# monniert/differentiable-blocksworld

Measured on AMD Instinct MI355X. Metric: rendered views/sec (fwd+bwd) per node, DTU 400x300 K=10 blocks, higher is better.
Workload: dtype f32; 1 GPU; DTU-scan24-like synthetic: 49 views/GPU/step, 400x300, 10 superquadric blocks + ground + sky dome, faces_per_pixel=10, 256^2 textures, coarse phase (sigma=1e-4, opacity noise, decimated textures), MSE+parsimony+TV+overlap, Adam; LPIPS excluded; views_per_gpu=49, n_blocks=10, faces_per_pixel=10, txt_size=256, parallelism=one GPU: all views on it, no collective, nranks=1

## Files before the change

differentiable-blocksworld_amd/csrc/model_ops.hip:

```cpp
#include "dbw_common.h"
#include "model_math.h"
#include "rng_math.h"
#include "texture_body.h"
#include "step_kernels.h"
#include "../../include/dbw_hip.h"

using namespace dbw;

namespace {

__device__ __forceinline__ int dense_index(const int *keep, int k) {
    if (!keep) return k;
    int c = 0;
    for (int i = 0; i < k; ++i) c += keep[i] != 0;
    return c;
}

__global__ __launch_bounds__(64) void sq_blocks_fwd_kernel(const float *sq_eps, const float *S, const float *R6, const float *T,
                                                           const float *trig, const int *keep, int dense, int Kb, int nv, float ratio,
                                                           float scale_min, float S_world, const float *Rw, const float *Tw,
                                                           float *verts) {
    const int k = blockIdx.x;
    if (keep && !keep[k]) {
        if (!dense)
// ... 31 lines not shown
        float loc[3], de1[3], de2[3];
        parametric_sq_point(trig[o], trig[plane + o], trig[2 * plane + o], trig[3 * plane + o], p.e1, p.e2, ratio, loc, de1, de2);
        float gv[3];
        pose_bwd(p, loc, S_world, Rw, gverts + ((long long)ko * nv + v) * 3, acc, gv);
        acc[0] += gv[0] * de1[0] + gv[1] * de1[1] + gv[2] * de1[2];
        acc[1] += gv[0] * de2[0] + gv[1] * de2[1] + gv[2] * de2[2];
    }
#pragma unroll
    for (int i = 0; i < 17; ++i) acc[i] = wave_sum(acc[i]);
    if (threadIdx.x == 0) finish_pose_grads(p, S, k, acc, g_sq_eps, g_S, g_R6, g_T);
}

__global__ __launch_bounds__(64) void posed_mesh_fwd_kernel(const float *base, int nv, const float *R6, const float *T,
                                                            float S_world, const float *Rw, const float *Tw, float *verts) {
    Pose p;
    load_pose(nullptr, nullptr, R6, T, 0, 0.f, p);
    for (int v = blockIdx.x * 64 + threadIdx.x; v < nv; v += gridDim.x * 64)
        pose_fwd(p, base + (long long)v * 3, S_world, Rw, Tw, verts + (long long)v * 3);
}

__global__ __launch_bounds__(64) void posed_mesh_bwd_kernel(const float *base, int nv, const float *R6, const float *T,
                                                            float S_world, const float *Rw, const float *gverts, float *g_R6,
                                                            float *g_T) {
    Pose p;
    load_pose(nullptr, nullptr, R6, T, 0, 0.f, p);
    float acc[17];
#pragma unroll
    for (int i = 0; i < 17; ++i) acc[i] = 0.f;
    for (int v = threadIdx.x; v < nv; v += 64) {
        float gv[3];
        pose_bwd(p, base + (long long)v * 3, S_world, Rw, gverts + (long long)v * 3, acc, gv);
    }
#pragma unroll
    for (int i = 0; i < 17; ++i) acc[i] = wave_sum(acc[i]);
    if (threadIdx.x == 0) finish_pose_grads(p, nullptr, 0, acc, nullptr, nullptr, g_R6, g_T);
}

constexpr int MAX_KB = 64;
constexpr int NG = 18;

struct BlockP {
    float e1, e2, sr[3], R[9], T[3], alpha;
};

struct OverlapShared { BlockP b[MAX_KB]; float g[MAX_KB * NG]; float red[4]; };
__device__ __forceinline__ void overlap_block(const float *u, unsigned long long seed, unsigned long long rng_step, int npts, const float *sq_eps,
                                              const float *S, const float *R6, const float *T, const float *alpha, int Kb, float ratio,
                                              float scale_min, float inv_temp, float thresh, float scale_over_P, float *loss, float *ws,
                                              OverlapShared &sh) {
    BlockP *s_b = sh.b;
    float *s_g = sh.g, *s_red = sh.red;
    for (int j = threadIdx.x; j < Kb; j += blockDim.x) {
        Pose p;
        load_pose(sq_eps, S, R6, T, j, scale_min, p);
        BlockP &b = s_b[j];
        b.e1 = p.e1; b.e2 = p.e2; b.alpha = alpha[j];
        for (int i = 0; i < 3; ++i) { b.sr[i] = p.S[i] * ratio; b.T[i] = p.T[i]; b.R[i] = p.rot.b1[i]; b.R[3 + i] = p.rot.b2[i]; b.R[6 + i] = p.rot.b3[i]; }
    }
// ... 354 lines not shown
```

differentiable-blocksworld_amd/csrc/project_clip.hip:

```cpp
#include "dbw_common.h"
#include "camera_math.h"
#include "shade_common.h"
#include "raster_bin.h"
#include "step_kernels.h"
#include "texture_body.h"
#include "../../include/dbw_hip.h"

using namespace dbw;

namespace {

constexpr int NT = 256;

__device__ __forceinline__ void store_tri(float *dst, f3 a, f3 b, f3 c) {
    dst[0] = a.x; dst[1] = a.y; dst[2] = a.z;
    dst[3] = b.x; dst[4] = b.y; dst[5] = b.z;
    dst[6] = c.x; dst[7] = c.y; dst[8] = c.z;
}

__global__ __launch_bounds__(NT) void project_clip_fwd_kernel(
    const float *__restrict__ verts, const int *__restrict__ faces, const float *__restrict__ R,
    const float *__restrict__ T, const float *__restrict__ Kmat, int V, int F, float eps, int zc_on, float zc,
    int persp, float *__restrict__ fvc, int *__restrict__ first_idx, int *__restrict__ num_faces,
    int *__restrict__ c2o, int *__restrict__ neighbor, int *__restrict__ code, float *__restrict__ cw) {
// ... 19 lines not shown
        const int prefix = __popcll(m1 & lower) + __popcll(m2 & lower);
        if (lane == 0) s_wcnt[wv] = __popcll(m1) + __popcll(m2);
        __syncthreads();
        int woff = 0, tot = 0;
#pragma unroll
        for (int w = 0; w < NT / DBW_WAVE; ++w) { const int c = s_wcnt[w]; if (w < wv) woff += c; tot += c; }
        const int slot = running + woff + prefix;
        if (emit >= 1) {
            const long long o = base_out + slot;
            store_tri(fvc + o * 9, cf.t0[0], cf.t0[1], cf.t0[2]);
            c2o[o] = f; neighbor[o] = emit == 2 ? (int)(o + 1) : -1; code[o] = cf.code0; cw[o * 2] = cf.w2; cw[o * 2 + 1] = cf.w3;
            if (emit == 2) {
                store_tri(fvc + (o + 1) * 9, cf.t1[0], cf.t1[1], cf.t1[2]);
                c2o[o + 1] = f; neighbor[o + 1] = (int)o; code[o + 1] = cf.code1; cw[(o + 1) * 2] = cf.w2; cw[(o + 1) * 2 + 1] = cf.w3;
            }
        }
        running += tot;
        __syncthreads();
    }
    if (tid == 0) { first_idx[b] = (int)base_out; num_faces[b] = running; }
}

constexpr int BWD_SLOTS = 8;
template <bool LDS_TABLE>
__device__ __forceinline__ void project_clip_bwd_body(
    const float *__restrict__ verts, const int *__restrict__ faces, const float *__restrict__ R,
    const float *__restrict__ T, const float *__restrict__ Kmat, int B, int V, int F, float eps, float zc, int persp,
    const int *__restrict__ num_faces, const int *__restrict__ c2o, const int *__restrict__ code,
    const float *__restrict__ cw, const float *__restrict__ gfvc, float *gverts, float *s_acc, int blk) {
    const int lane = threadIdx.x & 63;
    if (LDS_TABLE) {
        for (int i = threadIdx.x; i < V * 3; i += NT) s_acc[i] = 0.f;
        __syncthreads();
    }
    constexpr int WAVES = NT / DBW_WAVE, ITERS = LDS_TABLE ? BWD_SLOTS / WAVES : 1;
    for (int it = 0; it < ITERS; ++it) {
    const int j = LDS_TABLE ? blk * BWD_SLOTS + it * WAVES + (threadIdx.x >> 6) : blk * WAVES + (threadIdx.x >> 6);
    if (j >= 2 * F) break;
    for (int b0 = 0; b0 < B; b0 += DBW_WAVE) {
        const int b = b0 + lane;
        bool act = b < B && j < num_faces[b];
        const long long o = (long long)(act ? b : 0) * 2 * F + j;
        float g[9];
        if (act) {
            bool any = false;
#pragma unroll
            for (int i = 0; i < 9; ++i) { g[i] = gfvc[o * 9 + i]; any |= (g[i] != 0.f); }
            act = any;
        }
        int f = -1, vi[3] = {0, 0, 0};
        float gw[9] = {0.f, 0.f, 0.f, 0.f, 0.f, 0.f, 0.f, 0.f, 0.f};
        if (act) {
            Cam cam;
            load_cam(R, T, Kmat, b, cam);
            f = c2o[o];
            const int cd = code[o];
            vi[0] = faces[f * 3]; vi[1] = faces[f * 3 + 1]; vi[2] = faces[f * 3 + 2];
            f3 gv[3] = {{0.f, 0.f, 0.f}, {0.f, 0.f, 0.f}, {0.f, 0.f, 0.f}};
            const f3 ga{g[0], g[1], g[2]}, gb{g[3], g[4], g[5]}, gc{g[6], g[7], g[8]};
            if (cd < 0) {
                gv[0] = ga; gv[1] = gb; gv[2] = gc;
            } else {
                const int i1 = cd & 3, kind = cd >> 2;
                const f3 q0 = project(verts + (long long)vi[0] * 3, cam, eps).ndc, q1 = project(verts + (long long)vi[1] * 3, cam, eps).ndc,
                         q2 = project(verts + (long long)vi[2] * 3, cam, eps).ndc;
                const f3 P1 = i1 == 0 ? q0 : (i1 == 1 ? q1 : q2), P2 = i1 == 0 ? q1 : (i1 == 1 ? q2 : q0),
                         P3 = i1 == 0 ? q2 : (i1 == 1 ? q0 : q1);
                const float w2 = cw[o * 2], w3 = cw[o * 2 + 1];
                f3 g1{0.f, 0.f, 0.f}, g2{0.f, 0.f, 0.f}, g3{0.f, 0.f, 0.f};
                if (kind == 0) {
                    clip_point_bwd(P1, P2, zc, persp, w2, ga, g1, g2);
                    clip_point_bwd(P1, P3, zc, persp, w3, gb, g1, g3);
                    g1.x += gc.x; g1.y += gc.y; g1.z += gc.z;
                } else if (kind == 1) {
                    clip_point_bwd(P1, P2, zc, persp, w2, ga, g1, g2);
                    g2.x += gb.x; g2.y += gb.y; g2.z += gb.z;
                    clip_point_bwd(P1, P3, zc, persp, w3, gc, g1, g3);
                } else {
                    clip_point_bwd(P1, P3, zc, persp, w3, ga, g1, g3);
                    g2.x += gb.x; g2.y += gb.y; g2.z += gb.z;
                    g3.x += gc.x; g3.y += gc.y; g3.z += gc.z;
                }
                gv[0] = i1 == 0 ? g1 : (i1 == 1 ? g3 : g2);
                gv[1] = i1 == 0 ? g2 : (i1 == 1 ? g1 : g3);
                gv[2] = i1 == 0 ? g3 : (i1 == 1 ? g2 : g1);
            }
#pragma unroll
            for (int i = 0; i < 3; ++i)
                if (gv[i].x != 0.f || gv[i].y != 0.f || gv[i].z != 0.f) {
                    const f3 w = vertex_bwd(verts, vi[i], cam, eps, gv[i]);
                    gw[i * 3] = w.x; gw[i * 3 + 1] = w.y; gw[i * 3 + 2] = w.z;
                }
        }
        const unsigned long long am = __ballot(act);
        if (am == 0ull) continue;
        const int leader = __ffsll((long long)am) - 1;
        const int f0 = __shfl(f, leader, 64);
        if (__popcll(am) >= 4 && __ballot(act && f == f0) == am) {
            float s[9];
#pragma unroll
            for (int c = 0; c < 9; ++c) s[c] = wave_sum_dpp(gw[c]);
            if (lane == leader) {
#pragma unroll
                for (int c = 0; c < 9; ++c)
                    if (s[c] != 0.f) {
                        if (LDS_TABLE) atomicAdd(&s_acc[vi[c / 3] * 3 + (c % 3)], s[c]);
                        else unsafeAtomicAdd(gverts + (long long)vi[c / 3] * 3 + (c % 3), s[c]);
                    }
            }
        } else if (act) {
#pragma unroll
            for (int c = 0; c < 9; ++c)
                if (gw[c] != 0.f) {
                    if (LDS_TABLE) atomicAdd(&s_acc[vi[c / 3] * 3 + (c % 3)], gw[c]);
                    else unsafeAtomicAdd(gverts + (long long)vi[c / 3] * 3 + (c % 3), gw[c]);
                }
        }
    }
    }
    if (LDS_TABLE) {
        __syncthreads();
        for (int i = threadIdx.x; i < V * 3; i += NT) {
            const float v = s_acc[i];
            if (v != 0.f) unsafeAtomicAdd(gverts + i, v);
        }
    }
}

template <bool LDS_TABLE>
__global__ __launch_bounds__(NT) void project_clip_bwd_kernel(
    const float *__restrict__ verts, const int *__restrict__ faces, const float *__restrict__ R,
    const float *__restrict__ T, const float *__restrict__ Kmat, int B, int V, int F, float eps, float zc, int persp,
    const int *__restrict__ num_faces, const int *__restrict__ c2o, const int *__restrict__ code,
    const float *__restrict__ cw, const float *__restrict__ gfvc, float *__restrict__ gverts) {
    extern __shared__ float s_acc[];
    project_clip_bwd_body<LDS_TABLE>(verts, faces, R, T, Kmat, B, V, F, eps, zc, persp, num_faces, c2o, code, cw, gfvc, gverts, s_acc, blockIdx.x);
}

template <bool LDS_TABLE>
__global__ __launch_bounds__(NT) void clip_bwd_tex_kernel(const ClipBwdArgs C, const dbw_texture_set t, int nclip) {
    extern __shared__ float s_acc[];
    if ((int)blockIdx.x < nclip)
        project_clip_bwd_body<LDS_TABLE>(C.verts, C.faces, C.R, C.T, C.Kmat, C.B, C.V, C.F, C.eps, C.zc, C.persp, C.num_faces, C.c2o, C.code, C.cw, C.gfvc,
                                         C.gverts, s_acc, blockIdx.x);
    else
        texture_prep_bwd_body(t.texture, t.n, t.h, t.w, t.decim, t.grad_maps, t.grad_sig, t.grad_texture, (long long)blockIdx.x - nclip,
                              (long long)gridDim.x - nclip);
}

template <bool CACHED>
__global__ __launch_bounds__(NT) void scene_setup_kernel(const SceneSetupArgs A) {
    __shared__ int s_wcnt[NT / DBW_WAVE];
    extern __shared__ float s_ndc[];
    if (A.sync_flag && blockIdx.x == 0 && blockIdx.y == 0 && blockIdx.z == 0 && threadIdx.x == 0)
        __hip_atomic_store(A.sync_flag, A.sync_val, __ATOMIC_RELEASE, __HIP_MEMORY_SCOPE_AGENT);
    const SceneGeom &G = A.sc[A.scene0 + blockIdx.z];
    const int chunk = blockIdx.x, b = blockIdx.y, tid = threadIdx.x, lane = tid & 63, wv = tid >> 6;
    const int F = G.F, nchunks = (F + NT - 1) / NT;
    if (chunk >= nchunks) return;
    if (G.hdr && chunk == 0 && b == 0)
        for (int i = tid; i < G.nhdr; i += NT) G.hdr[i] = 0;
    Cam cam;
    load_cam(A.R, A.T, A.Kmat, b, cam);
    const long long base_out = (long long)b * 2 * F;
    const int f = chunk * NT + tid;
    int vi[3] = {0, 0, 0};
    if (f < F) { vi[0] = G.faces[f * 3]; vi[1] = G.faces[f * 3 + 1]; vi[2] = G.faces[f * 3 + 2]; }
    if (CACHED) {
        for (int v = tid; v < G.V; v += NT) {
            const f3 q = project(G.verts + (long long)v * 3, cam, G.cam_eps).ndc;
// ... 79 lines not shown
            srec[0] = sr;
        }
    }
}

}

int dbw::launch_clip_bwd_tex(const ClipBwdArgs &C, const dbw_texture_set &t, hipStream_t s) {
    DBW_REQUIRE(C.verts && C.faces && C.R && C.T && C.Kmat && C.num_faces && C.c2o && C.code && C.cw && C.gfvc && C.gverts, "null pointer");
    DBW_REQUIRE(C.B > 0 && C.V > 0 && C.F > 0, "bad size");
    DBW_REQUIRE(t.texture && t.grad_maps && t.grad_texture && t.n > 0 && t.h > 0 && t.w > 0 && t.decim >= 1, "bad texture set");
    const long long work = (long long)t.n * t.h * t.w * 3;
    long long ntex = (work + NT - 1) / NT;
    if (ntex > 4096) ntex = 4096;
    const bool table = (size_t)C.V * 3 * sizeof(float) <= 48 * 1024;
    const int nclip = table ? (2 * C.F + BWD_SLOTS - 1) / BWD_SLOTS : (2 * C.F + NT / DBW_WAVE - 1) / (NT / DBW_WAVE);
    if (table)
        hipLaunchKernelGGL(clip_bwd_tex_kernel<true>, dim3((unsigned)(nclip + ntex)), dim3(NT), (size_t)C.V * 3 * sizeof(float), s, C, t, nclip);
    else
        hipLaunchKernelGGL(clip_bwd_tex_kernel<false>, dim3((unsigned)(nclip + ntex)), dim3(NT), 0, s, C, t, nclip);
    return dbw_check_launch("clip_bwd_tex_kernel");
}

int dbw::launch_scene_setup(const SceneSetupArgs &A, hipStream_t s) {
    DBW_REQUIRE(A.R && A.T && A.Kmat && A.B > 0, "bad argument");
    int chunks = 0;
    DBW_REQUIRE(A.scene0 >= 0 && A.nscenes >= 1 && A.scene0 + A.nscenes <= 2, "bad scene range");
    for (int i = A.scene0; i < A.scene0 + A.nscenes; ++i) {
        const SceneGeom &G = A.sc[i];
        DBW_REQUIRE(G.verts && G.faces && G.fvc && G.first_idx && G.num_faces && G.c2o && G.neighbor && G.code && G.cw && G.bbox && G.recs, "null pointer");
        DBW_REQUIRE(G.V > 0 && G.F > 0 && (long long)A.B * 2 * G.F < 0x7fffffffLL && (!G.zc_on || G.zc > 0.f), "bad size / z_clip");
        DBW_REQUIRE(!G.srec || (G.face_uvs && G.face_map && G.map_desc), "null pointer");
        chunks = max(chunks, (G.F + NT - 1) / NT);
    }
    int vmax = 0;
    for (int i = A.scene0; i < A.scene0 + A.nscenes; ++i) vmax = max(vmax, A.sc[i].V);
    if ((size_t)vmax * 12 <= 40 * 1024)
        hipLaunchKernelGGL(scene_setup_kernel<true>, dim3((unsigned)chunks, (unsigned)A.B, (unsigned)A.nscenes), dim3(NT), (size_t)vmax * 12, s, A);
    else
        hipLaunchKernelGGL(scene_setup_kernel<false>, dim3((unsigned)chunks, (unsigned)A.B, (unsigned)A.nscenes), dim3(NT), 0, s, A);
    return dbw_check_launch("scene_setup_kernel");
}

extern "C" int dbw_project_clip_fwd(const float *verts_world, const int32_t *faces, const float *R, const float *T,
                                    const float *Kmat, int B, int V, int F, float eps, int z_clip_enabled,
                                    float z_clip, int perspective_correct, float *face_verts_c, int32_t *first_idx,
// ... 34 lines not shown
```

differentiable-blocksworld_amd/csrc/step_kernels.h:

```cpp
#pragma once
#include <hip/hip_runtime.h>
#include <stdint.h>

#include "../../include/dbw_hip.h"

namespace dbw {
struct RasterWorkspace;

constexpr int STEP_MAX_SETS = 4;
struct StepTextureSets { dbw_texture_set s[STEP_MAX_SETS]; };

struct PrologueArgs {
    StepTextureSets tex; int nsets;
    const float *alpha_logit, *noise;
    float noise_scale, thresh;
    int nb;
    float *alpha, *alpha_full;
    int *keep;
    unsigned long long seed, rng_step;
    const float *sq_eps, *S, *R6, *T, *trig;
    int nv;
    float ratio, scale_min, S_world;
    const float *Rw, *Tw;
    float *blk_verts;
// ... 41 lines not shown
    float pars_eps, pars_scale;
    float *loss_parsimony, *loss_overlap;
    float *g_sq_eps, *g_S, *g_R6, *g_T, *g_alpha_full;
    float *ws;
    unsigned *ticket;
};
int launch_regularisers(const RegulariserArgs &A, hipStream_t s);

struct BlocksTailArgs {
    const float *sq_eps, *S, *R6, *T, *sq_local; const int *keep; int nb, nv; float scale_min, S_world; const float *Rw;
    const float *g_verts;
    float *g_sq_eps, *g_S, *g_R6, *g_T;
    const float *alpha, *g_alpha_parts, *g_alpha_full; int alpha_parts; float *g_logit;
    const float *void_raised; float *void_flag;
};
int launch_blocks_tail(const BlocksTailArgs &A, hipStream_t s);

struct ClipBwdArgs {
    const float *verts; const int *faces; const float *R, *T, *Kmat; int B, V, F; float eps, zc; int persp;
    const int *num_faces, *c2o, *code; const float *cw, *gfvc; float *gverts;
};
int launch_clip_bwd_tex(const ClipBwdArgs &C, const dbw_texture_set &tex, hipStream_t s);

struct AdamTailArgs {
    float *param, *grad, *exp_avg, *exp_avg_sq; const int64_t *group_end; const float *lr; int ngroups;
    float beta1, beta2, eps; int step;
    void *zero_buf; int64_t zero_bytes, hole_begin, hole_end;
    dbw_texture_set tex[2]; int ntex;
    const float *void_raised; float *void_flag;
};
bool adam_tail_fits(const AdamTailArgs &A);
int launch_adam_tail(const AdamTailArgs &A, hipStream_t s);

struct EnvFoldHost {
    const RasterWorkspace *ws; const int *first_idx, *num_faces; const float *maps; float bg[3];
    int *p2f; float *uvj;
};
int render_fwd_fused_mse_fold(const float *face_verts_c, const int32_t *first_idx, const int32_t *num_faces, const int32_t *neighbor,
                              const int32_t *c2o, const int32_t *clip_code, const float *clip_w, int Fc_stride, const float *face_uvs,
                              const int32_t *face_map, const int32_t *map_desc, const float *maps, const float *faces_alpha, int alpha_len, int N,
                              int64_t F_total, int H, int W, int K, int F, float sigma, float blur_radius, int perspective_correct,
                              const float *background3, int32_t *pix_to_face, float *bary, float *dists, void *workspace, size_t workspace_bytes,
                              const float *target, float mse_scale, float *loss_partial, float *grad_fg, float *grad_env, const EnvFoldHost &fold,
                              float *rec_out, const float *grad_rec, hipStream_t stream);

int render_bwd_fused_signal(const int32_t *pix_to_face, const float *bary, const float *dists, const int32_t *c2o, const int32_t *clip_code,
// ... 9 lines not shown
```

differentiable-blocksworld_amd/csrc/train_step.hip:

```cpp
#include "dbw_common.h"
#include "raster_bin.h"
#include "step_kernels.h"
#include "../../include/dbw_hip.h"

#include <math.h>
#include <mutex>
#include <new>
#include <stdlib.h>
#include <string.h>

using namespace dbw;

namespace {

__global__ __launch_bounds__(256) void tile_target_kernel(const float *__restrict__ img, int B, int C, int H, int W, float *__restrict__ out) {
    const int tx = (W + 7) >> 3, ty = (H + 7) >> 3;
    const long long total = (long long)B * ty * tx * C * 64;
    for (long long i = (long long)blockIdx.x * blockDim.x + threadIdx.x; i < total; i += (long long)gridDim.x * blockDim.x) {
        const int lane = (int)(i & 63);
        long long r = i >> 6;
        const int c = (int)(r % C); r /= C;
        const int tix = (int)(r % tx); r /= tx;
        const int tiy = (int)(r % ty);
        const int n = (int)(r / ty);
// ... 237 lines not shown

struct dbw_step_plan {
    dbw_step_desc d;
    Layout L;
    char *ws;
    RasterWorkspace rw_e, rw_f;
    hipEvent_t ev_prologue, ev_scatter, ev_fg_fwd, ev_reg, ev_layout, ev_kernel_done, ev_blocks_ready, ev_env_done, ev_losses;
    hipStream_t stream_r, stream_env;
    unsigned long long runs;
    int bin_turn, bin_ready, uniform_ready;
    bool arena_clean;
    float *host_losses;
    bool losses_pending;
    bool phase1_done;
    bool cur_flags;
    bool profile, profiled;
    hipEvent_t ev_t[8];
    unsigned *sync_words;
    unsigned *host_timeouts, *host_timeouts_dev;
    unsigned sync_val[SYNC_FLAGS];
    int voided_runs;
    int force_timeout;
    bool last_tail;
};

extern "C" size_t dbw_train_step_workspace_bytes(const dbw_step_desc *desc) {
    if (check_desc(desc)) return 0;
    Layout L;
    make_layout(*desc, L);
    return L.total;
}

extern "C" dbw_step_plan *dbw_train_step_create(const dbw_step_desc *desc, void *workspace, size_t workspace_bytes) {
    if (check_desc(desc)) return nullptr;
    if (!workspace || ((uintptr_t)workspace & 255)) { dbw_set_error("dbw_train_step_create: the workspace must be 256-byte aligned"); return nullptr; }
    dbw_step_plan *p = new (std::nothrow) dbw_step_plan();
    if (!p) { dbw_set_error("dbw_train_step_create: out of host memory"); return nullptr; }
    p->d = *desc;
    make_layout(p->d, p->L);
    if (workspace_bytes < p->L.total) {
        dbw_set_error("dbw_train_step_create: workspace of %zu bytes, %zu needed", workspace_bytes, p->L.total);
        dbw_train_step_destroy(p);
        return nullptr;
    }
    p->ws = (char *)workspace;
    hipEvent_t *evs[] = {&p->ev_prologue, &p->ev_scatter, &p->ev_fg_fwd, &p->ev_reg, &p->ev_layout, &p->ev_kernel_done, &p->ev_blocks_ready, &p->ev_env_done, &p->ev_losses};
// ... 7 lines not shown
    }
    for (int i = 0; i < 8; ++i) p->host_losses[i] = 0.f;
    p->sync_words = nullptr;
    if (hipMalloc((void **)&p->sync_words, SYNC_WORDS * sizeof(unsigned)) != hipSuccess || hipMemset(p->sync_words, 0, SYNC_WORDS * sizeof(unsigned)) != hipSuccess) {
        dbw_set_error("dbw_train_step_create: hipMalloc failed");
        dbw_train_step_destroy(p);
        return nullptr;
    }
    for (unsigned &v : p->sync_val) v = 0;
    p->host_timeouts = nullptr; p->host_timeouts_dev = nullptr;
    if (hipHostMalloc((void **)&p->host_timeouts, 64, hipHostMallocMapped) != hipSuccess ||
        hipHostGetDevicePointer((void **)&p->host_timeouts_dev, p->host_timeouts, 0) != hipSuccess) {
        dbw_set_error("dbw_train_step_create: hipHostMalloc (mapped) failed");
        dbw_train_step_destroy(p);
        return nullptr;
    }
    *p->host_timeouts = 0u;
    p->profile = p->profiled = false;
    p->phase1_done = false;
    for (hipEvent_t &e : p->ev_t)
        if (hipEventCreate(&e) != hipSuccess) { dbw_set_error("dbw_train_step_create: hipEventCreate failed"); dbw_train_step_destroy(p); return nullptr; }
    p->runs = 0; p->cur_flags = false; p->voided_runs = 0; p->force_timeout = 0; p->bin_turn = 0; p->bin_ready = 0; p->uniform_ready = 0; p->arena_clean = false; p->losses_pending = false;
    p->last_tail = false;
    return p;
}

extern "C" void dbw_train_step_destroy(dbw_step_plan *p) {
    if (!p) return;
    hipEvent_t evs[] = {p->ev_prologue, p->ev_scatter, p->ev_fg_fwd, p->ev_reg, p->ev_layout, p->ev_kernel_done, p->ev_blocks_ready, p->ev_env_done, p->ev_losses};
    for (hipEvent_t e : evs) if (e) (void)hipEventDestroy(e);
    for (hipEvent_t e : p->ev_t) if (e) (void)hipEventDestroy(e);
    if (p->host_losses) (void)hipHostFree(p->host_losses);
    if (p->sync_words) (void)hipFree(p->sync_words);
    if (p->host_timeouts) (void)hipHostFree(p->host_timeouts);
    delete p;
}

extern "C" int64_t dbw_train_step_offset(const dbw_step_plan *p, int which) {
    if (!p) return -1;
    const Layout &L = p->L;
    switch (which) {
        case 0: return (int64_t)L.alpha;
        case 1: return (int64_t)L.alpha_full;
        case 2: return (int64_t)L.keep;
        case 3: return (int64_t)L.losses;
        case 4: return (int64_t)L.arena_begin;
// ... 315 lines not shown
    } else
    RC(dbw_render_fwd_fused_mse(FP(L.f.fvc), IP(L.f.first), IP(L.f.num), IP(L.f.nbr), IP(L.f.c2o), IP(L.f.code), FP(L.f.cw), 2 * Ff, d.block_face_uvs,
                                d.block_face_map, d.block_map_desc, FP(L.blk_maps), fa, alpha_len, B, Ftf, H, W, K, Ff, d.sigma, d.blur_radius,
                                d.perspective_correct, d.bg_fg, IP(L.p2f), FP(L.bary), FP(L.dists), ws + L.f.rws, L.f.rws_bytes, FP(L.img_e), target, mse_scale,
                                FP(L.part), FP(L.g_fg), FP(L.g_env), 2, 1, M));
    PROF(3, M);
    const bool seq = d.backward_order != 0 || (bins && !d.binned_concurrent);
    const bool fwd_signal_folded = flags && two;
    if (two && !fwd_signal_folded) RC(signal(M, F_FG_FWD, p->ev_fg_fwd));

    auto loss_values = [&](hipStream_t st) -> int {
        hipLaunchKernelGGL(loss_finish_kernel, dim3(LOSS_BLOCKS), dim3(256), 0, st, FP(L.part), (long long)B * L.tiles, mse_scale,
                           d.tv_value_scale != 0.f ? d.tv_value_scale : 1.f, vals, FP(L.losses));
        RC(dbw_check_launch("loss_finish_kernel"));
        if (two) RC(signal(st, F_REG, p->ev_reg));
        if (in->read_losses) {
            HIP_OK(hipMemcpyAsync(p->host_losses, FP(L.losses), 5 * sizeof(float), hipMemcpyDeviceToHost, st));
            HIP_OK(hipEventRecord(p->ev_losses, st));
            p->losses_pending = true;
        }
        return DBW_OK;
    };

    auto env_backward = [&](hipStream_t st) -> int {
        PROF(6, st);
        RC(dbw_render_bwd_fused(IP(L.p2f_e), FP(L.bary_e), FP(L.dists_e), IP(L.e.c2o), IP(L.e.code), FP(L.e.cw), 2 * Fe, d.env_face_uvs, d.env_face_map,
                                d.env_map_desc, FP(L.env_maps), nullptr, 0, B, H, W, 1, Fe, 0.f, d.bg_env, FP(L.g_env), FP(L.e.fvc), d.perspective_correct, 0,
                                FP(L.g_env_maps), nullptr, FP(L.g_fvc_e), 1, 3, nullptr, nullptr, nullptr, 0, nullptr, d.n_sky_faces, nullptr, 1, st));
        PROF(7, st);
        RC(dbw_project_clip_bwd(d.env_verts, d.env_faces, in->R, in->T, d.Kmat, B, Ve, Fe, d.cam_eps, d.z_clip, d.perspective_correct, IP(L.e.num),
                                IP(L.e.c2o), IP(L.e.code), FP(L.e.cw), FP(L.g_fvc_e), FP(L.g_env_verts), st));
        RC(dbw_posed_mesh_bwd(d.ground_base, d.n_ground_verts, d.R6_ground, d.T_ground, d.S_world, d.R_world, FP(L.g_env_verts) + (size_t)d.n_sky_verts * 3,
                              d.g_R6_ground, d.g_T_ground, st));
        if (defer || adam_tail) return DBW_OK;
        if (two) RC(await(st, F_REG, p->ev_reg));
        dbw_texture_set env_sets[2] = {sets[0], sets[2]};
        if (!tv) { env_sets[0].grad_sig = nullptr; env_sets[1].grad_sig = nullptr; }
        RC(dbw_texture_prep_bwd_sets(env_sets, 2, st));
        return DBW_OK;
    };
    auto side_after_fwd = [&]() -> int {
        if (two) {
            RC(await(Rg, F_FG_FWD, p->ev_fg_fwd));
            RC(loss_values(Rg));
        }
        if (two && !seq) {
            RC(await(E, F_FG_FWD, p->ev_fg_fwd));
            RC(env_backward(E));
            RC(signal(E, F_ENV_DONE, p->ev_env_done));
        }
        return DBW_OK;
    };
    if (!fwd_signal_folded) RC(side_after_fwd());

    if (bins && two) RC(await(M, F_LAYOUT, p->ev_layout));
    PROF(4, M);
    unsigned *bwd_flag = nullptr, bwd_val = 0;
    if (fwd_signal_folded) { bwd_flag = p->sync_words + F_FG_FWD; bwd_val = ++p->sync_val[F_FG_FWD]; }
    RC(render_bwd_fused_signal(IP(L.p2f), FP(L.bary), FP(L.dists), IP(L.f.c2o), IP(L.f.code), FP(L.f.cw), 2 * Ff, d.block_face_uvs, d.block_face_map,
                               d.block_map_desc, FP(L.blk_maps), fa, alpha_len, B, H, W, K, Ff, d.sigma, d.bg_fg, FP(L.g_fg), FP(L.f.fvc), d.perspective_correct, 1,
                               FP(L.g_blk_maps), coarse ? FP(L.g_fa) : nullptr, FP(L.g_fvc_f), d.decim_blocks > 1 ? 1 : 0, 2, bins ? d.block_bin_base : nullptr, cursor,
                               bins ? (void *)(ws + L.records) : nullptr, bins ? L.bin_cap : 0, blayout, 0, nullptr, 1, M, bwd_flag, bwd_val));
    PROF(5, M);
    if (fwd_signal_folded) RC(side_after_fwd());
    if (two && seq) {
        RC(signal(M, F_KERNEL_DONE, p->ev_kernel_done));
        RC(await(E, F_KERNEL_DONE, p->ev_kernel_done));
        RC(env_backward(E));
        RC(signal(E, F_ENV_DONE, p->ev_env_done));
    }
    if (bins) RC(dbw_texbin_reduce(d.block_bin_info, cursor, ws + L.records, L.bin_cap, blayout, d.n_bins, FP(L.g_blk_maps), M));
    if (adam_tail) RC(await(M, F_REG, p->ev_reg));
    const bool early_textures = two && !in->with_adam && !defer;
    auto blocks_textures = [&]() -> int {
        if (defer) return DBW_OK;
        dbw_texture_set blk = sets[1];
        if (!tv) blk.grad_sig = nullptr;
        RC(dbw_texture_prep_bwd_sets(&blk, 1, M));
        if (early_textures) RC(signal(M, F_BLOCKS_READY, p->ev_blocks_ready));
        return DBW_OK;
    };
    if (early_textures) {
        RC(await(M, F_REG, p->ev_reg));
        RC(blocks_textures());
    }
    const bool tail_merged = (d.fuse & 32) && !early_textures && !defer;
    if (!tail_merged)
        RC(dbw_project_clip_bwd(FP(L.blk_verts), d.block_faces, in->R, in->T, d.Kmat, B, Vf, Ff, d.cam_eps, d.z_clip, d.perspective_correct, IP(L.f.num),
                                IP(L.f.c2o), IP(L.f.code), FP(L.f.cw), FP(L.g_fvc_f), FP(L.g_blk_verts), M));
    if (!two) { RC(env_backward(M)); RC(loss_values(M)); }
    auto blocks_chain = [&]() -> int {
        if (tail_merged) {
            ClipBwdArgs C;
            C.verts = FP(L.blk_verts); C.faces = d.block_faces; C.R = in->R; C.T = in->T; C.Kmat = d.Kmat; C.B = B; C.V = Vf; C.F = Ff;
            C.eps = d.cam_eps; C.zc = d.z_clip; C.persp = d.perspective_correct;
            C.num_faces = IP(L.f.num); C.c2o = IP(L.f.c2o); C.code = IP(L.f.code); C.cw = FP(L.f.cw); C.gfvc = FP(L.g_fvc_f); C.gverts = FP(L.g_blk_verts);
            dbw_texture_set blk = sets[1];
            if (!tv) blk.grad_sig = nullptr;
            RC(launch_clip_bwd_tex(C, blk, M));
        } else if (!early_textures) RC(blocks_textures());
        if ((d.fuse & 8) && (d.fuse & 1)) {
            BlocksTailArgs A;
            memset(&A, 0, sizeof(A));
            A.sq_eps = d.sq_eps; A.S = d.S; A.R6 = d.R6; A.T = d.T; A.sq_local = FP(L.sq_local); A.keep = IP(L.keep); A.nb = nb; A.nv = nv;
            A.scale_min = d.scale_min; A.S_world = d.S_world; A.Rw = d.R_world; A.g_verts = FP(L.g_blk_verts);
            A.g_sq_eps = d.g_sq_eps; A.g_S = d.g_S; A.g_R6 = d.g_R6; A.g_T = d.g_T;
            A.alpha = FP(L.alpha); A.g_alpha_parts = coarse ? FP(L.g_fa) : nullptr; A.alpha_parts = 64; A.g_alpha_full = FP(L.g_alpha_full); A.g_logit = d.g_alpha_logit;
            if (!adam_tail) { A.void_raised = void_raised; A.void_flag = void_flag; }
            RC(launch_blocks_tail(A, M));
        } else {
            RC(dbw_sq_blocks_bwd(d.sq_eps, d.S, d.R6, d.T, d.trig, IP(L.keep), 0, nb, nv, d.ratio_block_scene, d.scale_min, d.S_world, d.R_world, FP(L.g_blk_verts),
                                 d.g_sq_eps, d.g_S, d.g_R6, d.g_T, M));
            RC(dbw_block_alpha_bwd(FP(L.alpha), IP(L.keep), coarse ? FP(L.g_fa) : nullptr, 64, FP(L.g_alpha_full), nb, d.g_alpha_logit, M));
            hipLaunchKernelGGL(void_latch_kernel, dim3(1), dim3(1), 0, M, (const float *)void_raised, void_flag);
            RC(dbw_check_launch("void_latch_kernel"));
        }
        return DBW_OK;
    };
    if (adam_tail) RC(blocks_chain());
    if (two) RC(await(M, F_ENV_DONE, p->ev_env_done));
    if (two && defer) RC(await(M, F_REG, p->ev_reg));
    if (!adam_tail) RC(blocks_chain());

    if (adam_tail) {
        T.tex[0] = sets[0]; T.tex[1] = sets[2];
        if (!tv) { T.tex[0].grad_sig = nullptr; T.tex[1].grad_sig = nullptr; }
        RC(launch_adam_tail(T, M));
        p->arena_clean = true;
        p->last_tail = true;
    } else if (in->with_adam) {
        p->last_tail = false;
        RC(dbw_adam_step_groups(d.flat_param, d.flat_grad, d.exp_avg, d.exp_avg_sq, d.group_end, in->lr, 2, in->beta1, in->beta2, in->adam_eps, in->adam_step,
                                ws + L.arena_begin, (int64_t)(L.arena_end - L.arena_begin), void_flag, M));
        p->arena_clean = true;
    }
    if (bins) { p->bin_turn = 1 - p->bin_turn; p->bin_ready = 1; }
    p->runs += 1;
    p->profiled = p->profile;
    return DBW_OK;
// ... 44 lines not shown
    unsigned w[3] = {0u, 0u, 0u};
    if (hipDeviceSynchronize() != hipSuccess || hipMemcpy(w, p->sync_words + SYNC_TIMEOUT_SLOT - 3, sizeof(w), hipMemcpyDeviceToHost) != hipSuccess) {
        dbw_set_error("dbw_debug_train_step_last_timeout: copy failed");
        return DBW_ERR_LAUNCH;
    }
    out3[0] = (int)w[0] - 1; out3[1] = (int)w[1]; out3[2] = (int)w[2];
    return DBW_OK;
}
extern "C" int dbw_debug_train_step_counters(dbw_step_plan *p, unsigned *seen12, unsigned *asked12) {
    DBW_REQUIRE(p && seen12 && asked12, "null pointer");
    unsigned first = 0u;
    if (hipDeviceSynchronize() != hipSuccess || hipMemcpy(&first, p->sync_words + SYNC_TIMEOUT_SLOT - 3, sizeof(first), hipMemcpyDeviceToHost) != hipSuccess ||
        hipMemcpy(seen12, p->sync_words + (first ? SYNC_TIMEOUT_SLOT + 1 : 0), SYNC_FLAGS * sizeof(unsigned), hipMemcpyDeviceToHost) != hipSuccess) {
        dbw_set_error("dbw_debug_train_step_counters: copy failed");
        return DBW_ERR_LAUNCH;
    }
    for (int i = 0; i < SYNC_FLAGS; ++i) asked12[i] = p->sync_val[i];
    return DBW_OK;
}
extern "C" int dbw_train_step_voided_runs(const dbw_step_plan *p) { return p ? p->voided_runs + (*(volatile unsigned *)p->host_timeouts != 0u ? 1 : 0) : -1; }

extern "C" int dbw_debug_train_step_last_tail(const dbw_step_plan *p) { return p ? (p->last_tail ? 1 : 0) : -1; }

extern "C" int64_t dbw_train_step_void_flag_offset(const dbw_step_plan *p) { return p ? (int64_t)p->L.losses + 7 * (int64_t)sizeof(float) : -1; }

extern "C" int dbw_train_step_sync_timeouts(dbw_step_plan *p) {
    if (!p) return -1;
    unsigned n = 0;
    if (hipDeviceSynchronize() != hipSuccess || hipMemcpy(&n, p->sync_words + SYNC_TIMEOUT_SLOT, sizeof(n), hipMemcpyDeviceToHost) != hipSuccess) return -1;
    return (int)n;
}

extern "C" int dbw_train_step_profile(dbw_step_plan *p, int on) {
    DBW_REQUIRE(p, "null pointer");
    p->profile = on != 0;
    p->profiled = false;
    return DBW_OK;
}

extern "C" int dbw_train_step_kernel_times(dbw_step_plan *p, float *out4_ms) {
    DBW_REQUIRE(p && out4_ms, "null pointer");
    DBW_REQUIRE(p->profiled, "no profiled run: dbw_train_step_profile(plan, 1), then a run");
    for (int k = 0; k < 4; ++k) {
        HIP_OK(hipEventSynchronize(p->ev_t[2 * k + 1]));
        HIP_OK(hipEventElapsedTime(out4_ms + k, p->ev_t[2 * k], p->ev_t[2 * k + 1]));
    }
// ... 3 lines not shown
```

Baseline: 78800 views/s.

## Fuse ground clip backward with pose backward via last-block ticket tail kernel

Adds a ground_tail_kernel that runs clip backward only over ground faces, scanning clip slots from the end of each view's list. It accumulates ground vertex gradients in LDS, flushes them with atomics, and lets the last workgroup (chosen by a ticket) compute the ground pose gradients and raise the env-done sync word. This replaces the full env project_clip_bwd plus a separate posed_mesh_bwd launch, which cuts launches and skips sky-face work. The blocks chain is also split so block clip backward and block texture work launch as separate kernels rather than the merged tail. In exchange it adds ticket and fence ordering, relies on ground faces sitting at the end of each view's clip list, and is limited to grounds whose vertex gradients fit in 48 KB of LDS.

```diff
diff --git a/differentiable-blocksworld_amd/csrc/model_ops.hip b/differentiable-blocksworld_amd/csrc/model_ops.hip
--- a/differentiable-blocksworld_amd/csrc/model_ops.hip
+++ b/differentiable-blocksworld_amd/csrc/model_ops.hip
@@ -1,5 +1,6 @@
 #include "dbw_common.h"
 #include "model_math.h"
+#include "pose_body.h"
 #include "rng_math.h"
 #include "texture_body.h"
 #include "step_kernels.h"
@@ -77,18 +78,7 @@
 __global__ __launch_bounds__(64) void posed_mesh_bwd_kernel(const float *base, int nv, const float *R6, const float *T,
                                                             float S_world, const float *Rw, const float *gverts, float *g_R6,
                                                             float *g_T) {
-    Pose p;
-    load_pose(nullptr, nullptr, R6, T, 0, 0.f, p);
-    float acc[17];
-#pragma unroll
-    for (int i = 0; i < 17; ++i) acc[i] = 0.f;
-    for (int v = threadIdx.x; v < nv; v += 64) {
-        float gv[3];
-        pose_bwd(p, base + (long long)v * 3, S_world, Rw, gverts + (long long)v * 3, acc, gv);
-    }
-#pragma unroll
-    for (int i = 0; i < 17; ++i) acc[i] = wave_sum(acc[i]);
-    if (threadIdx.x == 0) finish_pose_grads(p, nullptr, 0, acc, nullptr, nullptr, g_R6, g_T);
+    posed_mesh_bwd_wave<false>(base, nv, R6, T, S_world, Rw, gverts, g_R6, g_T, threadIdx.x);
 }
 
 constexpr int MAX_KB = 64;
diff --git a/differentiable-blocksworld_amd/csrc/pose_body.h b/differentiable-blocksworld_amd/csrc/pose_body.h
--- /dev/null
+++ b/differentiable-blocksworld_amd/csrc/pose_body.h
@@ -0,0 +1,30 @@
+#pragma once
+#include "dbw_common.h"
+#include "model_math.h"
+
+namespace dbw {
+
+template <bool SHARED>
+__device__ __forceinline__ void posed_mesh_bwd_wave(const float *base, int nv, const float *R6, const float *T, float S_world, const float *Rw,
+                                                    const float *gverts, float *g_R6, float *g_T, int lane) {
+    Pose p;
+    load_pose(nullptr, nullptr, R6, T, 0, 0.f, p);
+    float acc[17];
+#pragma unroll
+    for (int i = 0; i < 17; ++i) acc[i] = 0.f;
+    for (int v = lane; v < nv; v += 64) {
+        float gv[3];
+        if (SHARED) {
+            float g[3];
+#pragma unroll
+            for (int i = 0; i < 3; ++i) g[i] = __hip_atomic_load(gverts + (long long)v * 3 + i, __ATOMIC_RELAXED, __HIP_MEMORY_SCOPE_AGENT);
+            pose_bwd(p, base + (long long)v * 3, S_world, Rw, g, acc, gv);
+        } else
+            pose_bwd(p, base + (long long)v * 3, S_world, Rw, gverts + (long long)v * 3, acc, gv);
+    }
+#pragma unroll
+    for (int i = 0; i < 17; ++i) acc[i] = wave_sum(acc[i]);
+    if (lane == 0) finish_pose_grads(p, nullptr, 0, acc, nullptr, nullptr, g_R6, g_T);
+}
+
+}
diff --git a/differentiable-blocksworld_amd/csrc/project_clip.hip b/differentiable-blocksworld_amd/csrc/project_clip.hip
--- a/differentiable-blocksworld_amd/csrc/project_clip.hip
+++ b/differentiable-blocksworld_amd/csrc/project_clip.hip
@@ -1,5 +1,6 @@
 #include "dbw_common.h"
 #include "camera_math.h"
+#include "pose_body.h"
 #include "shade_common.h"
 #include "raster_bin.h"
 #include "step_kernels.h"
@@ -65,6 +66,81 @@
 }
 
 constexpr int BWD_SLOTS = 8;
+
+__device__ __forceinline__ void clip_slot_bwd(const float *__restrict__ verts, const int *__restrict__ faces, const float *__restrict__ R,
+                                              const float *__restrict__ T, const float *__restrict__ Kmat, int b, long long o, float eps, float zc,
+                                              int persp, const int *__restrict__ c2o, const int *__restrict__ code, const float *__restrict__ cw,
+                                              const float (&g)[9], int &f, int (&vi)[3], float (&gw)[9]) {
+    Cam cam;
+    load_cam(R, T, Kmat, b, cam);
+    f = c2o[o];
+    const int cd = code[o];
+    vi[0] = faces[f * 3]; vi[1] = faces[f * 3 + 1]; vi[2] = faces[f * 3 + 2];
+    f3 gv[3] = {{0.f, 0.f, 0.f}, {0.f, 0.f, 0.f}, {0.f, 0.f, 0.f}};
+    const f3 ga{g[0], g[1], g[2]}, gb{g[3], g[4], g[5]}, gc{g[6], g[7], g[8]};
+    if (cd < 0) {
+        gv[0] = ga; gv[1] = gb; gv[2] = gc;
+    } else {
+        const int i1 = cd & 3, kind = cd >> 2;
+        const f3 q0 = project(verts + (long long)vi[0] * 3, cam, eps).ndc, q1 = project(verts + (long long)vi[1] * 3, cam, eps).ndc,
+                 q2 = project(verts + (long long)vi[2] * 3, cam, eps).ndc;
+        const f3 P1 = i1 == 0 ? q0 : (i1 == 1 ? q1 : q2), P2 = i1 == 0 ? q1 : (i1 == 1 ? q2 : q0),
+                 P3 = i1 == 0 ? q2 : (i1 == 1 ? q0 : q1);
+        const float w2 = cw[o * 2], w3 = cw[o * 2 + 1];
+        f3 g1{0.f, 0.f, 0.f}, g2{0.f, 0.f, 0.f}, g3{0.f, 0.f, 0.f};
+        if (kind == 0) {
+            clip_point_bwd(P1, P2, zc, persp, w2, ga, g1, g2);
+            clip_point_bwd(P1, P3, zc, persp, w3, gb, g1, g3);
+            g1.x += gc.x; g1.y += gc.y; g1.z += gc.z;
+        } else if (kind == 1) {
+            clip_point_bwd(P1, P2, zc, persp, w2, ga, g1, g2);
+            g2.x += gb.x; g2.y += gb.y; g2.z += gb.z;
+            clip_point_bwd(P1, P3, zc, persp, w3, gc, g1, g3);
+        } else {
+            clip_point_bwd(P1, P3, zc, persp, w3, ga, g1, g3);
+            g2.x += gb.x; g2.y += gb.y; g2.z += gb.z;
+            g3.x += gc.x; g3.y += gc.y; g3.z += gc.z;
+        }
+        gv[0] = i1 == 0 ? g1 : (i1 == 1 ? g3 : g2);
+        gv[1] = i1 == 0 ? g2 : (i1 == 1 ? g1 : g3);
+        gv[2] = i1 == 0 ? g3 : (i1 == 1 ? g2 : g1);
+    }
+#pragma unroll
+    for (int i = 0; i < 3; ++i)
+        if (gv[i].x != 0.f || gv[i].y != 0.f || gv[i].z != 0.f) {
+            const f3 w = vertex_bwd(verts, vi[i], cam, eps, gv[i]);
+            gw[i * 3] = w.x; gw[i * 3 + 1] = w.y; gw[i * 3 + 2] = w.z;
+        }
+}
+
+template <bool LDS_TABLE>
+__device__ __forceinline__ void clip_slot_accumulate(bool act, int f, const int (&vi)[3], const float (&gw)[9], int lane, float *acc, int vbase) {
+    const unsigned long long am = __ballot(act);
+    if (am == 0ull) return;
+    const int leader = __ffsll((long long)am) - 1;
+    const int f0 = __shfl(f, leader, 64);
+    if (__popcll(am) >= 4 && __ballot(act && f == f0) == am) {
+        float s[9];
+#pragma unroll
+        for (int c = 0; c < 9; ++c) s[c] = wave_sum_dpp(gw[c]);
+        if (lane == leader) {
+#pragma unroll
+            for (int c = 0; c < 9; ++c)
+                if (s[c] != 0.f) {
+                    if (LDS_TABLE) atomicAdd(&acc[(vi[c / 3] - vbase) * 3 + (c % 3)], s[c]);
+                    else unsafeAtomicAdd(acc + (long long)(vi[c / 3] - vbase) * 3 + (c % 3), s[c]);
+                }
+        }
+    } else if (act) {
+#pragma unroll
+        for (int c = 0; c < 9; ++c)
+            if (gw[c] != 0.f) {
+                if (LDS_TABLE) atomicAdd(&acc[(vi[c / 3] - vbase) * 3 + (c % 3)], gw[c]);
+                else unsafeAtomicAdd(acc + (long long)(vi[c / 3] - vbase) * 3 + (c % 3), gw[c]);
+            }
+    }
+}
+
 template <bool LDS_TABLE>
 __device__ __forceinline__ void project_clip_bwd_body(
     const float *__restrict__ verts, const int *__restrict__ faces, const float *__restrict__ R,
@@ -93,72 +169,8 @@
         }
         int f = -1, vi[3] = {0, 0, 0};
         float gw[9] = {0.f, 0.f, 0.f, 0.f, 0.f, 0.f, 0.f, 0.f, 0.f};
-        if (act) {
-            Cam cam;
-            load_cam(R, T, Kmat, b, cam);
-            f = c2o[o];
-            const int cd = code[o];
-            vi[0] = faces[f * 3]; vi[1] = faces[f * 3 + 1]; vi[2] = faces[f * 3 + 2];
-            f3 gv[3] = {{0.f, 0.f, 0.f}, {0.f, 0.f, 0.f}, {0.f, 0.f, 0.f}};
-            const f3 ga{g[0], g[1], g[2]}, gb{g[3], g[4], g[5]}, gc{g[6], g[7], g[8]};
-            if (cd < 0) {
-                gv[0] = ga; gv[1] = gb; gv[2] = gc;
-            } else {
-                const int i1 = cd & 3, kind = cd >> 2;
-                const f3 q0 = project(verts + (long long)vi[0] * 3, cam, eps).ndc, q1 = project(verts + (long long)vi[1] * 3, cam, eps).ndc,
-                         q2 = project(verts + (long long)vi[2] * 3, cam, eps).ndc;
-                const f3 P1 = i1 == 0 ? q0 : (i1 == 1 ? q1 : q2), P2 = i1 == 0 ? q1 : (i1 == 1 ? q2 : q0),
-                         P3 = i1 == 0 ? q2 : (i1 == 1 ? q0 : q1);
-                const float w2 = cw[o * 2], w3 = cw[o * 2 + 1];
-                f3 g1{0.f, 0.f, 0.f}, g2{0.f, 0.f, 0.f}, g3{0.f, 0.f, 0.f};
-                if (kind == 0) {
-                    clip_point_bwd(P1, P2, zc, persp, w2, ga, g1, g2);
-                    clip_point_bwd(P1, P3, zc, persp, w3, gb, g1, g3);
-                    g1.x += gc.x; g1.y += gc.y; g1.z += gc.z;
-                } else if (kind == 1) {
-                    clip_point_bwd(P1, P2, zc, persp, w2, ga, g1, g2);
-                    g2.x += gb.x; g2.y += gb.y; g2.z += gb.z;
-                    clip_point_bwd(P1, P3, zc, persp, w3, gc, g1, g3);
-                } else {
-                    clip_point_bwd(P1, P3, zc, persp, w3, ga, g1, g3);
-                    g2.x += gb.x; g2.y += gb.y; g2.z += gb.z;
-                    g3.x += gc.x; g3.y += gc.y; g3.z += gc.z;
-                }
-                gv[0] = i1 == 0 ? g1 : (i1 == 1 ? g3 : g2);
-                gv[1] = i1 == 0 ? g2 : (i1 == 1 ? g1 : g3);
-                gv[2] = i1 == 0 ? g3 : (i1 == 1 ? g2 : g1);
-            }
-#pragma unroll
-            for (int i = 0; i < 3; ++i)
-                if (gv[i].x != 0.f || gv[i].y != 0.f || gv[i].z != 0.f) {
-                    const f3 w = vertex_bwd(verts, vi[i], cam, eps, gv[i]);
-                    gw[i * 3] = w.x; gw[i * 3 + 1] = w.y; gw[i * 3 + 2] = w.z;
-                }
-        }
-        const unsigned long long am = __ballot(act);
-        if (am == 0ull) continue;
-        const int leader = __ffsll((long long)am) - 1;
-        const int f0 = __shfl(f, leader, 64);
-        if (__popcll(am) >= 4 && __ballot(act && f == f0) == am) {
-            float s[9];
-#pragma unroll
-            for (int c = 0; c < 9; ++c) s[c] = wave_sum_dpp(gw[c]);
-            if (lane == leader) {
-#pragma unroll
-                for (int c = 0; c < 9; ++c)
-                    if (s[c] != 0.f) {
-                        if (LDS_TABLE) atomicAdd(&s_acc[vi[c / 3] * 3 + (c % 3)], s[c]);
-                        else unsafeAtomicAdd(gverts + (long long)vi[c / 3] * 3 + (c % 3), s[c]);
-                    }
-            }
-        } else if (act) {
-#pragma unroll
-            for (int c = 0; c < 9; ++c)
-                if (gw[c] != 0.f) {
-                    if (LDS_TABLE) atomicAdd(&s_acc[vi[c / 3] * 3 + (c % 3)], gw[c]);
-                    else unsafeAtomicAdd(gverts + (long long)vi[c / 3] * 3 + (c % 3), gw[c]);
-                }
-        }
+        if (act) clip_slot_bwd(verts, faces, R, T, Kmat, b, o, eps, zc, persp, c2o, code, cw, g, f, vi, gw);
+        clip_slot_accumulate<LDS_TABLE>(act, f, vi, gw, lane, LDS_TABLE ? s_acc : gverts, 0);
     }
     }
     if (LDS_TABLE) {
@@ -189,6 +201,58 @@
     else
         texture_prep_bwd_body(t.texture, t.n, t.h, t.w, t.decim, t.grad_maps, t.grad_sig, t.grad_texture, (long long)blockIdx.x - nclip,
                               (long long)gridDim.x - nclip);
+}
+
+__global__ __launch_bounds__(NT) void ground_tail_kernel(const GroundTailArgs A) {
+    extern __shared__ float s_acc[];
+    __shared__ int s_last;
+    constexpr int WAVES = NT / DBW_WAVE;
+    const int lane = threadIdx.x & 63, nacc = A.n_ground_verts * 3;
+    for (int i = threadIdx.x; i < nacc; i += NT) s_acc[i] = 0.f;
+    __syncthreads();
+    for (int t = blockIdx.x * WAVES + (threadIdx.x >> 6); t < 2 * A.n_ground_faces; t += gridDim.x * WAVES)
+        for (int b0 = 0; b0 < A.B; b0 += DBW_WAVE) {
+            const int b = b0 + lane;
+            const int j = b < A.B ? min(A.num_faces[b], 2 * A.F) - 1 - t : -1;
+            bool act = j >= 0;
+            const long long o = act ? (long long)b * 2 * A.F + j : 0;
+            if (act) { const int f = A.c2o[o]; act = f >= A.n_sky_faces && f < A.F; }
+            float g[9];
+            if (act) {
+                bool any = false;
+#pragma unroll
+                for (int i = 0; i < 9; ++i) { g[i] = A.gfvc[o * 9 + i]; any |= (g[i] != 0.f); }
+                act = any;
+            }
+            int f = -1, vi[3] = {0, 0, 0};
+            float gw[9] = {0.f, 0.f, 0.f, 0.f, 0.f, 0.f, 0.f, 0.f, 0.f};
+            if (act) {
+                clip_slot_bwd(A.verts, A.faces, A.R, A.T, A.Kmat, b, o, A.eps, A.zc, A.persp, A.c2o, A.code, A.cw, g, f, vi, gw);
+                if ((unsigned)(vi[0] - A.n_sky_verts) >= (unsigned)A.n_ground_verts || (unsigned)(vi[1] - A.n_sky_verts) >= (unsigned)A.n_ground_verts ||
+                    (unsigned)(vi[2] - A.n_sky_verts) >= (unsigned)A.n_ground_verts) {
+                    act = false;
+#pragma unroll
+                    for (int c = 0; c < 9; ++c) gw[c] = 0.f;
+                }
+            }
+            clip_slot_accumulate<true>(act, f, vi, gw, lane, s_acc, A.n_sky_verts);
+        }
+    __syncthreads();
+    for (int i = threadIdx.x; i < nacc; i += NT) {
+        const float v = s_acc[i];
+        if (v != 0.f) unsafeAtomicAdd(A.g_verts + i, v);
+    }
+    __threadfence();
+    __syncthreads();
+    if (threadIdx.x == 0) s_last = atomicAdd(A.ticket, 1u) == gridDim.x - 1 ? 1 : 0;
+    __syncthreads();
+    if (!s_last || threadIdx.x >= DBW_WAVE) return;
+    __threadfence();
+    posed_mesh_bwd_wave<true>(A.ground_base, A.n_ground_verts, A.R6, A.T_ground, A.S_world, A.Rw, A.g_verts, A.g_R6, A.g_T, lane);
+    if (lane == 0) {
+        __hip_atomic_store(A.ticket, 0u, __ATOMIC_RELAXED, __HIP_MEMORY_SCOPE_AGENT);
+        if (A.sync_flag) __hip_atomic_store(A.sync_flag, A.sync_val, __ATOMIC_RELEASE, __HIP_MEMORY_SCOPE_AGENT);
+    }
 }
 
 template <bool CACHED>
@@ -314,6 +378,35 @@
     return dbw_check_launch("clip_bwd_tex_kernel");
 }
 
+int dbw::launch_ground_tail(const GroundTailArgs &A, int workgroups, hipStream_t s) {
+    DBW_REQUIRE(A.verts && A.faces && A.R && A.T && A.Kmat && A.num_faces && A.c2o && A.code && A.cw && A.gfvc && A.g_verts && A.ticket, "null pointer");
+    DBW_REQUIRE(A.ground_base && A.R6 && A.T_ground && A.Rw && A.g_R6 && A.g_T, "null pointer");
+    DBW_REQUIRE(A.B > 0 && A.n_sky_faces >= 0 && A.n_ground_faces > 0 && A.F == A.n_sky_faces + A.n_ground_faces && A.n_sky_verts >= 0 && A.n_ground_verts > 0,
+                "bad size");
+    DBW_REQUIRE((size_t)A.n_ground_verts * 12 <= 48 * 1024, "the ground's vertex gradients are kept in 48 KB of LDS");
+    const int full = (2 * A.n_ground_faces + NT / DBW_WAVE - 1) / (NT / DBW_WAVE);
+    DBW_REQUIRE(workgroups >= 0 && workgroups <= full, "bad grid");
+    hipLaunchKernelGGL(ground_tail_kernel, dim3((unsigned)(workgroups ? workgroups : full)), dim3(NT), (size_t)A.n_ground_verts * 12, s, A);
+    return dbw_check_launch("ground_tail_kernel");
+}
+
+extern "C" int dbw_debug_ground_tail(const float *env_verts, const int32_t *env_faces, const float *R, const float *T, const float *Kmat, int B, int n_sky_verts,
+                                     int n_ground_verts, int n_sky_faces, int n_ground_faces, float eps, float z_clip, int perspective_correct,
+                                     const int32_t *num_faces, const int32_t *c2o, const int32_t *clip_code, const float *clip_w,
+                                     const float *grad_face_verts_c, const float *ground_base, const float *R6, const float *T_ground, float S_world,
+                                     const float *R_world, float *ws, float *g_R6, float *g_T, int workgroups, dbw_stream_t stream) {
+    DBW_REQUIRE(ws && n_ground_verts > 0, "null workspace");
+    GroundTailArgs A;
+    A.verts = env_verts; A.faces = env_faces; A.R = R; A.T = T; A.Kmat = Kmat; A.B = B; A.F = n_sky_faces + n_ground_faces;
+    A.n_sky_faces = n_sky_faces; A.n_ground_faces = n_ground_faces; A.n_sky_verts = n_sky_verts; A.n_ground_verts = n_ground_verts;
+    A.eps = eps; A.zc = z_clip; A.persp = perspective_correct;
+    A.num_faces = num_faces; A.c2o = c2o; A.code = clip_code; A.cw = clip_w; A.gfvc = grad_face_verts_c;
+    A.g_verts = ws; A.ticket = (unsigned *)(ws + (size_t)n_ground_verts * 3);
+    A.ground_base = ground_base; A.R6 = R6; A.T_ground = T_ground; A.S_world = S_world; A.Rw = R_world; A.g_R6 = g_R6; A.g_T = g_T;
+    A.sync_flag = nullptr; A.sync_val = 0;
+    return launch_ground_tail(A, workgroups, (hipStream_t)stream);
+}
+
 int dbw::launch_scene_setup(const SceneSetupArgs &A, hipStream_t s) {
     DBW_REQUIRE(A.R && A.T && A.Kmat && A.B > 0, "bad argument");
     int chunks = 0;
diff --git a/differentiable-blocksworld_amd/csrc/step_kernels.h b/differentiable-blocksworld_amd/csrc/step_kernels.h
--- a/differentiable-blocksworld_amd/csrc/step_kernels.h
+++ b/differentiable-blocksworld_amd/csrc/step_kernels.h
@@ -87,6 +87,19 @@
 };
 int launch_clip_bwd_tex(const ClipBwdArgs &C, const dbw_texture_set &tex, hipStream_t s);
 
+struct GroundTailArgs {
+    const float *verts; const int *faces; const float *R, *T, *Kmat;
+    int B, F, n_sky_faces, n_ground_faces, n_sky_verts, n_ground_verts;
+    float eps, zc; int persp;
+    const int *num_faces, *c2o, *code; const float *cw, *gfvc;
+    float *g_verts;
+    unsigned *ticket;
+    const float *ground_base, *R6, *T_ground; float S_world; const float *Rw;
+    float *g_R6, *g_T;
+    unsigned *sync_flag; unsigned sync_val;
+};
+int launch_ground_tail(const GroundTailArgs &A, int workgroups, hipStream_t s);
+
 struct AdamTailArgs {
     float *param, *grad, *exp_avg, *exp_avg_sq; const int64_t *group_end; const float *lr; int ngroups;
     float beta1, beta2, eps; int step;
diff --git a/differentiable-blocksworld_amd/csrc/train_step.hip b/differentiable-blocksworld_amd/csrc/train_step.hip
--- a/differentiable-blocksworld_amd/csrc/train_step.hip
+++ b/differentiable-blocksworld_amd/csrc/train_step.hip
@@ -283,6 +283,7 @@
     int voided_runs;
     int force_timeout;
     bool last_tail;
+    int tail_form;
 };
 
 extern "C" size_t dbw_train_step_workspace_bytes(const dbw_step_desc *desc) {
@@ -336,6 +337,7 @@
         if (hipEventCreate(&e) != hipSuccess) { dbw_set_error("dbw_train_step_create: hipEventCreate failed"); dbw_train_step_destroy(p); return nullptr; }
     p->runs = 0; p->cur_flags = false; p->voided_runs = 0; p->force_timeout = 0; p->bin_turn = 0; p->bin_ready = 0; p->uniform_ready = 0; p->arena_clean = false; p->losses_pending = false;
     p->last_tail = false;
+    p->tail_form = 1;
     return p;
 }
 
@@ -697,16 +699,36 @@
         return DBW_OK;
     };
 
+    const int tail_form = p->tail_form;
+    const bool ground_tail = tail_form != 0 && adam_tail && (size_t)d.n_ground_verts * 12 <= 48 * 1024;
+    bool env_word_stored = false;
     auto env_backward = [&](hipStream_t st) -> int {
         PROF(6, st);
         RC(dbw_render_bwd_fused(IP(L.p2f_e), FP(L.bary_e), FP(L.dists_e), IP(L.e.c2o), IP(L.e.code), FP(L.e.cw), 2 * Fe, d.env_face_uvs, d.env_face_map,
                                 d.env_map_desc, FP(L.env_maps), nullptr, 0, B, H, W, 1, Fe, 0.f, d.bg_env, FP(L.g_env), FP(L.e.fvc), d.perspective_correct, 0,
                                 FP(L.g_env_maps), nullptr, FP(L.g_fvc_e), 1, 3, nullptr, nullptr, nullptr, 0, nullptr, d.n_sky_faces, nullptr, 1, st));
         PROF(7, st);
-        RC(dbw_project_clip_bwd(d.env_verts, d.env_faces, in->R, in->T, d.Kmat, B, Ve, Fe, d.cam_eps, d.z_clip, d.perspective_correct, IP(L.e.num),
-                                IP(L.e.c2o), IP(L.e.code), FP(L.e.cw), FP(L.g_fvc_e), FP(L.g_env_verts), st));
-        RC(dbw_posed_mesh_bwd(d.ground_base, d.n_ground_verts, d.R6_ground, d.T_ground, d.S_world, d.R_world, FP(L.g_env_verts) + (size_t)d.n_sky_verts * 3,
-                              d.g_R6_ground, d.g_T_ground, st));
+        if (ground_tail) {
+            GroundTailArgs G;
+            memset(&G, 0, sizeof(G));
+            G.verts = d.env_verts; G.faces = d.env_faces; G.R = in->R; G.T = in->T; G.Kmat = d.Kmat; G.B = B; G.F = Fe;
+            G.n_sky_faces = d.n_sky_faces; G.n_ground_faces = d.n_ground_faces; G.n_sky_verts = d.n_sky_verts; G.n_ground_verts = d.n_ground_verts;
+            G.eps = d.cam_eps; G.zc = d.z_clip; G.persp = d.perspective_correct;
+            G.num_faces = IP(L.e.num); G.c2o = IP(L.e.c2o); G.code = IP(L.e.code); G.cw = FP(L.e.cw); G.gfvc = FP(L.g_fvc_e);
+            G.g_verts = FP(L.g_env_verts) + (size_t)d.n_sky_verts * 3; G.ticket = (unsigned *)(ws + L.tickets) + 1;
+            G.ground_base = d.ground_base; G.R6 = d.R6_ground; G.T_ground = d.T_ground; G.S_world = d.S_world; G.Rw = d.R_world;
+            G.g_R6 = d.g_R6_ground; G.g_T = d.g_T_ground;
+            if (two && flags && (defer || adam_tail)) {
+                G.sync_flag = p->sync_words + F_ENV_DONE; G.sync_val = ++p->sync_val[F_ENV_DONE];
+                env_word_stored = true;
+            }
+            RC(launch_ground_tail(G, tail_form == 2 ? 1 : 0, st));
+        } else {
+            RC(dbw_project_clip_bwd(d.env_verts, d.env_faces, in->R, in->T, d.Kmat, B, Ve, Fe, d.cam_eps, d.z_clip, d.perspective_correct, IP(L.e.num),
+                                    IP(L.e.c2o), IP(L.e.code), FP(L.e.cw), FP(L.g_fvc_e), FP(L.g_env_verts), st));
+            RC(dbw_posed_mesh_bwd(d.ground_base, d.n_ground_verts, d.R6_ground, d.T_ground, d.S_world, d.R_world, FP(L.g_env_verts) + (size_t)d.n_sky_verts * 3,
+                                  d.g_R6_ground, d.g_T_ground, st));
+        }
         if (defer || adam_tail) return DBW_OK;
         if (two) RC(await(st, F_REG, p->ev_reg));
         dbw_texture_set env_sets[2] = {sets[0], sets[2]};
@@ -722,7 +744,7 @@
         if (two && !seq) {
             RC(await(E, F_FG_FWD, p->ev_fg_fwd));
             RC(env_backward(E));
-            RC(signal(E, F_ENV_DONE, p->ev_env_done));
+            if (!env_word_stored) RC(signal(E, F_ENV_DONE, p->ev_env_done));
         }
         return DBW_OK;
     };
@@ -742,7 +764,7 @@
         RC(signal(M, F_KERNEL_DONE, p->ev_kernel_done));
         RC(await(E, F_KERNEL_DONE, p->ev_kernel_done));
         RC(env_backward(E));
-        RC(signal(E, F_ENV_DONE, p->ev_env_done));
+        if (!env_word_stored) RC(signal(E, F_ENV_DONE, p->ev_env_done));
     }
     if (bins) RC(dbw_texbin_reduce(d.block_bin_info, cursor, ws + L.records, L.bin_cap, blayout, d.n_bins, FP(L.g_blk_maps), M));
     if (adam_tail) RC(await(M, F_REG, p->ev_reg));
@@ -764,8 +786,13 @@
         RC(dbw_project_clip_bwd(FP(L.blk_verts), d.block_faces, in->R, in->T, d.Kmat, B, Vf, Ff, d.cam_eps, d.z_clip, d.perspective_correct, IP(L.f.num),
                                 IP(L.f.c2o), IP(L.f.code), FP(L.f.cw), FP(L.g_fvc_f), FP(L.g_blk_verts), M));
     if (!two) { RC(env_backward(M)); RC(loss_values(M)); }
+    const bool split_chain = adam_tail && tail_merged && tail_form != 0;
     auto blocks_chain = [&]() -> int {
-        if (tail_merged) {
+        if (split_chain) {
+            if (tail_form == 3) RC(blocks_textures());
+            RC(dbw_project_clip_bwd(FP(L.blk_verts), d.block_faces, in->R, in->T, d.Kmat, B, Vf, Ff, d.cam_eps, d.z_clip, d.perspective_correct, IP(L.f.num),
+                                    IP(L.f.c2o), IP(L.f.code), FP(L.f.cw), FP(L.g_fvc_f), FP(L.g_blk_verts), M));
+        } else if (tail_merged) {
             ClipBwdArgs C;
             C.verts = FP(L.blk_verts); C.faces = d.block_faces; C.R = in->R; C.T = in->T; C.Kmat = d.Kmat; C.B = B; C.V = Vf; C.F = Ff;
             C.eps = d.cam_eps; C.zc = d.z_clip; C.persp = d.perspective_correct;
@@ -790,6 +817,7 @@
             hipLaunchKernelGGL(void_latch_kernel, dim3(1), dim3(1), 0, M, (const float *)void_raised, void_flag);
             RC(dbw_check_launch("void_latch_kernel"));
         }
+        if (split_chain && tail_form != 3) RC(blocks_textures());
         return DBW_OK;
     };
     if (adam_tail) RC(blocks_chain());
@@ -880,6 +908,19 @@
 
 extern "C" int dbw_debug_train_step_last_tail(const dbw_step_plan *p) { return p ? (p->last_tail ? 1 : 0) : -1; }
 
+extern "C" int dbw_debug_train_step_set_tail_form(dbw_step_plan *p, int form) {
+    if (!p || form < 0 || form > 3) return DBW_ERR_INVALID;
+    p->tail_form = form;
+    return DBW_OK;
+}
+
+extern "C" int dbw_debug_train_step_env_clip_offsets(const dbw_step_plan *p, int64_t *out5) {
+    if (!p || !out5) return DBW_ERR_INVALID;
+    out5[0] = (int64_t)p->L.e.first; out5[1] = (int64_t)p->L.e.num; out5[2] = (int64_t)p->L.e.c2o; out5[3] = (int64_t)p->L.e.code;
+    out5[4] = 2 * (int64_t)p->L.Fe;
+    return DBW_OK;
+}
+
 extern "C" int64_t dbw_train_step_void_flag_offset(const dbw_step_plan *p) { return p ? (int64_t)p->L.losses + 7 * (int64_t)sizeof(float) : -1; }
 
 extern "C" int dbw_train_step_sync_timeouts(dbw_step_plan *p) {
```

Result: no change. 79360 views/s, median of 4 (+0.7%).
